# szpajder/dumpvdl2

Hardware: AMD Instinct MI355X
Metric: IQ MS/s demodulated end-to-end (higher is better)
Workload: dtype f32

## Files before the change

dumpvdl2_amd/csrc/kernels.h:

```cpp
#pragma once
#include <hip/hip_runtime.h>
#include <type_traits>
#include "vdl2_core.h"
#include "design.h"

#ifndef VDL2_K1_UNROLL
#define VDL2_K1_UNROLL 5
#endif

#ifndef VDL2_K1_WAVES_PER_EU
#define VDL2_K1_WAVES_PER_EU 3
#endif

namespace vdl2 {

constexpr int kK1Unroll = VDL2_K1_UNROLL;
typedef float v2f __attribute__((ext_vector_type(2)));
typedef float v4f __attribute__((ext_vector_type(4)));

#ifndef VDL2_REF_PRIO
#define VDL2_REF_PRIO 3
#endif
#ifndef VDL2_K1_PRIO
#define VDL2_K1_PRIO 0
// ... 789 lines not shown
			const float4 ts = seg ? a.seg_end[(size_t)c * a.nseg_cap + seg - 1] : a.carry_in[c];
			const float *Pp = bf.Ppow[len];
			e.x += Pp[0] * ts.x + Pp[1] * ts.z; e.y += Pp[0] * ts.y + Pp[1] * ts.w;
			e.z += Pp[2] * ts.x + Pp[3] * ts.z; e.w += Pp[2] * ts.y + Pp[3] * ts.w;
		}
		a.carry_out[c] = e;
	}
}

__global__ void k_carry(K1Args a, void *carry_out, uint32_t nrem) {
	const uint32_t i = threadIdx.x;
	if(i >= nrem) return;
	const int64_t s = (int64_t)(a.nlogical - nrem) + i;
	if(a.fmt == 1) {
		const uint32_t *p = (s < (int64_t)a.ncarry) ? (const uint32_t *)a.carry + s : (const uint32_t *)a.in + (s - a.ncarry);
		((uint32_t *)carry_out)[i] = *p;
	} else {
		const uint16_t *p = (s < (int64_t)a.ncarry) ? (const uint16_t *)a.carry + s : (const uint16_t *)a.in + (s - a.ncarry);
		((uint16_t *)carry_out)[i] = *p;
	}
}

__device__ __forceinline__ void reset_out_ctl(OutCtl *ctl, uint32_t k5_waves) {
	ctl->nbursts = 0; ctl->overflow = 0; ctl->nvalid = 0; ctl->pool_out_used = 0;
	ctl->nframes = burst_reserve_initial_frames(k5_waves); ctl->pool_used = burst_reserve_initial_pool(k5_waves);
}
__global__ void k_reset_ctl(OutCtl *ctl, uint32_t k5_waves) { reset_out_ctl(ctl, k5_waves); }

struct K3Args {
	const cf32 *y; cf32 *pf; uint64_t *cand; uint64_t *flag; const Tables *tab;
	int64_t nbase, k1;
	uint32_t cap, mask;
	int32_t wpl;
	OutCtl *ctl; uint32_t k5_waves;
	RefChan *ref; RefChan refv; float max_ppm; const float *ppm_thr; int32_t ref_on; uint32_t *rq_n, *rq_flag; RefBad *rq_bad; ScanReq *pq; uint32_t pq_cap; uint32_t *rq_flag2;
};

#ifndef VDL2_K3_SHARE
#define VDL2_K3_SHARE 8
#endif
constexpr int kK3Share = VDL2_K3_SHARE, kK3Threads = 320, kK3Tile = kK3Threads * kK3Share;
static_assert(kK3Tile == kK3Threads * kK3Share && kK3Tile % 64 == 0 && kK3Threads % 10 == 0 && (kK3Tile / 64) % (kK3Threads / 64) == 0, "screen tile");

__global__ __launch_bounds__(kK3Threads) void k_sync_screen(K3Args a) {
	if(blockIdx.x == 0 && blockIdx.y == 0 && threadIdx.x == 0 && a.rq_n) a.rq_n[3] = 0u;
	__shared__ float tile[kK3Tile + 150];
	__shared__ uint8_t verdict[kK3Tile];
	const int c = blockIdx.y, tid = threadIdx.x;
	const int64_t nblk = a.nbase + (int64_t)blockIdx.x * kK3Tile;
	const cf32 *y = a.y + (size_t)c * a.cap;
	constexpr int kFull = (kK3Tile + 150) / kK3Threads, kRest = (kK3Tile + 150) % kK3Threads;
	if(nblk >= 150 && nblk + kK3Tile <= a.k1) {
		const uint32_t r0 = (uint32_t)(nblk - 150) + tid;
		cf32 v[kFull + 1];
		#pragma unroll
		for(int k = 0; k <= kFull; k++) if(k < kFull || tid < kRest) v[k] = y[(r0 + kK3Threads * k) & a.mask];
		#pragma unroll
		for(int k = 0; k <= kFull; k++) if(k < kFull || tid < kRest) tile[tid + kK3Threads * k] = phase_fast(v[k]);
	} else {
		for(int j = tid; j < kK3Tile + 150; j += kK3Threads) {
			const int64_t t = nblk - 150 + j;
			tile[j] = (t < 0 || t >= a.k1) ? 0.f : phase_fast(y[(uint32_t)t & a.mask]);
		}
	}
	__syncthreads();
	const int s0 = 10 * kK3Share * (tid / 10) + tid % 10;
	constexpr int kEarlyPh = kScreenEarly + kK3Share - 1;
	float ph[kEarlyPh], d[kEarlyPh];
	#pragma unroll
	for(int k = 0; k < kEarlyPh; k++) ph[k] = tile[s0 + 10 * k];
	#pragma unroll
	for(int k = 1; k < kEarlyPh; k++) d[k] = ph[k] - ph[k - 1];
	#pragma unroll
	for(int q = 0; q < kK3Share; q++) {
		ScreenAcc acc;
		screen_begin(acc);
		screen_taps(&d[q], 1, kScreenEarly, acc);
		float ps = screen_value(acc, kScreenEarly);
		if(__any(ps < kScreenEarlyThr)) {
			float pl[kPreamble - kScreenEarly + 1], dl[kPreamble];
			#pragma unroll
			for(int j = 0; j <= kPreamble - kScreenEarly; j++) pl[j] = tile[s0 + 10 * (q + kScreenEarly - 1 + j)];
			#pragma unroll
			for(int j = 0; j < kPreamble - kScreenEarly; j++) dl[kScreenEarly + j] = pl[j + 1] - pl[j];
			screen_taps(dl, kScreenEarly, kPreamble, acc);
			ps = screen_value(acc, kPreamble);
		}
		verdict[s0 + 10 * q] = !(ps >= kScreenThr);
	}
	__syncthreads();
	#pragma unroll
	for(int j = 0; j < (kK3Tile / 64) / (kK3Threads / 64); j++) {
		const int word = (tid >> 6) * ((kK3Tile / 64) / (kK3Threads / 64)) + j;
		const int64_t n = nblk + 64 * word + (tid & 63);
		const unsigned long long bits = __ballot(n < a.k1 && verdict[64 * word + (tid & 63)] != 0);
		if((tid & 63) == 0 && n < a.k1) a.flag[(size_t)c * (a.cap >> 6) + ((uint32_t)(n >> 6) & (a.mask >> 6))] = bits;
	}
}

constexpr int kK3bWordsPerLane = 4;
template<bool FULL>
__global__ __launch_bounds__(256, 4) void k_sync_exact4(K3Args a) {
	if(blockIdx.x == 0 && blockIdx.y == 0 && threadIdx.x == 0) { reset_out_ctl(a.ctl, a.k5_waves); if(a.ref) *a.ref = a.refv; if(a.rq_n) { a.rq_n[0] = 0u; a.rq_n[1] = 0u; a.rq_n[2] = 0u; a.rq_n[4] = 0u; a.rq_n[5] = 0u; a.rq_n[6] = 0u; } }
	if(blockIdx.x == 0 && threadIdx.x == 0 && a.rq_flag) { a.rq_flag[blockIdx.y] = 0u; a.rq_bad[blockIdx.y].n = 0u; if(a.rq_flag2) a.rq_flag2[blockIdx.y] = 0u; }
	constexpr int kBack = 160, kSpan = kBack + 64;
	__shared__ float psh[4][64 + 6], fsh[4][64 + 6], esh[4][64 + 6], ash[4][64 + 6], bsh[4][64 + 6];
	__shared__ float phs[4][kSpan], e2s[4][kSpan];
	__shared__ uint64_t s_need[4][64 * kK3bWordsPerLane];
	__shared__ uint8_t s_fprev[4][64 * kK3bWordsPerLane];
	__shared__ uint16_t s_list[4][64 * kK3bWordsPerLane];
	const int c = blockIdx.y, lane = threadIdx.x & 63, wave = threadIdx.x >> 6;
	const cf32 *y = a.y + (size_t)c * a.cap;
	const uint64_t *flag = a.flag + (size_t)c * (a.cap >> 6);
	uint64_t *cand = a.cand + (size_t)c * (a.cap >> 6);
	const uint32_t wmask = a.mask >> 6;
	const Tables &T = *a.tab;
	const bool ref_on = a.ref != nullptr && a.ref_on != 0;
	const float ppm_thr = ref_on ? a.ppm_thr[c] : 0.f;
	const int64_t w0 = a.nbase >> 6, w1 = (a.k1 + 63) >> 6;
	const int64_t wb = w0 + ((int64_t)blockIdx.x * 4 + wave) * (64 * a.wpl);
	int nwork = 0;
	for(int g = 0; g < a.wpl; g++) {
		const int64_t w = wb + 64 * g + lane;
		uint64_t need = 0, fprev = 0, fpp = 0, f0 = 0;
		if(w < w1) {
			f0 = flag[(uint32_t)w & wmask];
			fprev = w > 0 ? flag[(uint32_t)(w - 1) & wmask] : 0ull;
			fpp = w > 1 ? flag[(uint32_t)(w - 2) & wmask] : 0ull;
			const uint64_t fnext = w + 1 < w1 ? flag[(uint32_t)(w + 1) & wmask] : 0ull;
			need = f0 | (f0 << 3) | (f0 >> 3) | (fprev >> 61) | (fnext << 61);
			const int64_t base = w << 6;
			if(a.k1 - 3 < base + 64) {
				const int64_t lo = a.k1 - 3 - base;
				need |= lo <= 0 ? ~0ull : (~0ull << lo);
			}
			if(a.k1 < base + 64) need &= (a.k1 - base <= 0) ? 0ull : (~0ull >> (64 - (a.k1 - base)));
			if(need == 0) cand[(uint32_t)w & wmask] = 0;
		}
		const uint64_t need_prev = fprev | (fprev << 3) | (fprev >> 3) | (fpp >> 61) | (f0 << 61);
		s_need[wave][64 * g + lane] = need; s_fprev[wave][64 * g + lane] = (uint8_t)(need_prev >> 58);
		const unsigned long long busy = __ballot(need != 0);
		if(need != 0) s_list[wave][nwork + __builtin_popcountll(busy & ((1ull << lane) - 1ull))] = (uint16_t)(64 * g + lane);
		nwork += __builtin_popcountll(busy);
	}
	WAVE_SYNC();
	float *ps = psh[wave], *fs = fsh[wave], *es = esh[wave], *as = ash[wave], *bs = bsh[wave], *ph = phs[wave], *e2 = e2s[wave];
	#pragma unroll 1
	for(int it = 0; it < nwork; it++) {
		const int idx = (int)s_list[wave][it];
		const uint64_t needj = s_need[wave][idx];
		const uint32_t fprevj = s_fprev[wave][idx] & 63u;
		const int64_t wj = wb + idx, r0 = (wj << 6) - kBack;
		{
			cf32 yv[4]; bool in[4];
			#pragma unroll
			for(int k = 0; k < 4; k++) {
				const int64_t t = r0 + lane + 64 * k;
				in[k] = 64 * k + lane < kSpan && t >= 0 && t < a.k1;
				yv[k] = in[k] ? y[(uint32_t)t & a.mask] : cf32{0.f, 0.f};
			}
			#pragma unroll
			for(int k = 0; k < 4; k++) if(64 * k + lane < kSpan) {
				ph[64 * k + lane] = in[k] ? phase_of(yv[k]) : 0.f;
				e2[64 * k + lane] = in[k] ? yv[k].re * yv[k].re + yv[k].im * yv[k].im : -1.f;
			}
		}
		ps[6 + lane] = kPherrBig; if(lane < 6) ps[lane] = kPherrBig;
		WAVE_SYNC();
		if(ref_on) {
			float ev[4];
			#pragma unroll
			for(int k = 0; k < 4; k++) {
				const int i = 64 * k + lane;
				ev[k] = 0.f;
				if(i >= 3 && i < kSpan) {
					const float m0 = e2[i], m1 = e2[i - 1], m2 = e2[i - 2], m3 = e2[i - 3];
					ev[k] = m0 < 0.f ? 0.f : ref_eps2_of(m0, fmaxf(m1, 0.f), fmaxf(m2, 0.f), fmaxf(m3, 0.f));
				}
			}
			WAVE_SYNC();
			#pragma unroll
			for(int k = 0; k < 4; k++) if(64 * k + lane < kSpan) e2[64 * k + lane] = ev[k];
			WAVE_SYNC();
		}
		#pragma unroll 1
		for(int round = 0; round < 2; round++) {
			const int bit = round == 0 ? lane : lane - 6;
			const bool todo = round == 0 ? ((needj >> lane) & 1ull) != 0 : (lane < 6 && ((fprevj >> lane) & 1u) && (wj << 6) + bit >= 0);
			if(todo) {
				const int i0 = bit + kBack - 150;
				float p[kPreamble];
				#pragma unroll
				for(int i = 0; i < kPreamble; i++) p[i] = ph[i0 + 10 * i];
				float pv, fv, E = 0.f, pa, pb;
				if(ref_on) sync_metric_ref(p, e2 + i0, 10, T, pv, fv, E, pa, pb, FULL);
				else { sync_metric(p, T, pv, fv); pa = pb = pv; }
				ps[6 + bit] = pv; fs[6 + bit] = fv; es[6 + bit] = E; as[6 + bit] = pa; bs[6 + bit] = pb;
			}
		}
		WAVE_SYNC();
		const int64_t n = (wj << 6) + lane;
		const float p0 = ps[6 + lane], p3 = ps[3 + lane], p6 = ps[lane];
		int vd = 0;
		if(n >= 3 && n < a.k1) {
			if(!ref_on) vd = is_candidate(p3, p0) ? 1 : 0;
			else vd = ref_candidate_verdict(ref_pherr_range(p0, as[6 + lane], bs[6 + lane], es[6 + lane]), ref_pherr_range(p3, as[3 + lane], bs[3 + lane], es[3 + lane]), fs[3 + lane], es[3 + lane],
			                                ref_pherr_range(p6, as[lane], bs[lane], es[lane]), a.max_ppm, ppm_thr);
		}
		if((needj >> lane) & 1ull) a.pf[(size_t)c * a.cap + ((uint32_t)n & a.mask)] = cf32{ (vd & 2) ? -p0 : p0, fs[6 + lane] };
		const unsigned long long bits = __ballot((vd & 1) != 0);
		if(lane == 0) cand[(uint32_t)wj & wmask] = bits;
		if(a.pq) {
			const unsigned long long mk = __ballot((vd & 2) != 0 && ((needj >> lane) & 1ull) != 0);
			if(mk && lane == 0) {
				const int64_t nf = (wj << 6) + __builtin_ctzll(mk), nl = (wj << 6) + 63 - __builtin_clzll(mk);
				int64_t lo = (nf - kRefPre) & ~255ll, hi = (nl + kRefPost) | 255; if(lo < 0) lo = 0; if(hi > a.k1 - 1) hi = a.k1 - 1;
				const uint32_t i = atomicAdd(a.rq_n + 3, 1u);
				if(i < a.pq_cap) a.pq[i] = ScanReq{ c, REF_CANDIDATE, lo, hi };
			}
		}
		WAVE_SYNC();
	}
}

struct K4Args {
	const cf32 *y; const cf32 *pf; const uint64_t *cand; const Tables *tab;
	WalkState *ws; unsigned long long *cnt; Burst *bursts; uint32_t *nb_chan; uint32_t cap_bursts_chan; OutCtl *ctl; const uint32_t *freq;
	EvalChunk *log; uint32_t *nlog; uint32_t cap_log;
	int64_t k_end; float max_ppm; uint32_t cap, mask; int32_t chan_first, nchan;
	const float *ppm_thr;
	RefChan *ref;
	uint32_t ref_launch;
	RefReq *rq; uint32_t *rq_n; uint32_t rq_cap; uint32_t *rq_flag; WalkState *ws_snap; unsigned long long *cnt_snap; RefBad *rq_bad; int32_t ref_pre;
	int32_t force_again;
	WalkState *ws_tmp; unsigned long long *cnt_tmp; WalkState *ws_snap_next; unsigned long long *cnt_snap_next; uint32_t *rq_flag2, *rq_flag2_next;
	int32_t force_mismatch;
};

__global__ __launch_bounds__(64, 4) void k_walk(K4Args a) {
	__shared__ WalkShared sh;
	const int c = blockIdx.x;
	ChanView v{ a.y + (size_t)c * a.cap, a.pf + (size_t)c * a.cap, a.cand + (size_t)c * (a.cap >> 6), a.mask, a.ref, c, a.ref_launch, a.rq, a.rq_n, a.rq_cap, a.rq_flag, a.rq_bad ? a.rq_bad + c : nullptr, a.ref_pre != 0 };
	EvalLog lg{ a.log + (size_t)c * a.cap_log, a.nlog + c };
	walk_channel(c, a.freq[c], a.max_ppm, a.ppm_thr[c], a.k_end, *a.tab, v, &a.ws[c], a.cnt + (size_t)c * kNumCounters,
	             a.bursts + (size_t)c * a.cap_bursts_chan, a.cap_bursts_chan, a.nb_chan + c, a.ctl, lg, sh, WalkSnap{ a.rq ? a.ws_snap : nullptr, a.cnt_snap });
}

__global__ __launch_bounds__(64, 4) void k_ref_verify(K4Args a) {
	__shared__ float lds[64];
	const uint32_t nreq = *a.rq_n < a.rq_cap ? *a.rq_n : a.rq_cap;
	if(a.force_again && blockIdx.x == 0) for(int c = (int)threadIdx.x; c < a.nchan; c += 64) a.rq_flag[c] = 1u;
	for(uint32_t i = blockIdx.x; i < nreq; i += gridDim.x) {
		const RefReq r = a.rq[i];
		const int c = r.chan;
		ChanView v{ a.y + (size_t)c * a.cap, a.pf + (size_t)c * a.cap, a.cand + (size_t)c * (a.cap >> 6), a.mask, a.ref, c, a.ref_launch + 2u };
// ... 576 lines not shown
```

dumpvdl2_amd/csrc/vdl2hip.hip:

```cpp
#include <hip/hip_runtime.h>
#include <hip/hip_ext.h>
#include <algorithm>
#include <cstdio>
#include <cstdlib>
#include <cstring>
#include <memory>
#include <mutex>
#include <new>
#include <string>
#include <vector>
#include "../../include/vdl2hip.h"
#include "kernels.h"
#include "tables.h"

using namespace vdl2;

static_assert(VDL2HIP_NUM_COUNTERS == kNumCounters, "counter enum out of sync");

namespace {

struct HostFrame {
	OutFrame f;
	std::shared_ptr<std::vector<uint8_t>> pool;
	const uint8_t *octets() const { return pool && f.pool_off + f.len <= pool->size() ? pool->data() + f.pool_off : nullptr; }
// ... 47 lines not shown
	vdl2hip_cfg cfg{};
	int C = 0, chan_first = 0, os = 0, fmt = 0, run = kRun, cr = 1;
	bool specialised = false;
	std::vector<uint32_t> freqs, dphi;
	LpfCoeffs lpf{};
	BlockForm bf{};
	hipStream_t stream = nullptr;
	BlockForm *d_bf = nullptr; Lut4 *d_lut = nullptr; Tables *d_tab = nullptr;
	uint32_t *d_dphi = nullptr, *d_freq = nullptr; float *d_ppmthr = nullptr;
	uint8_t *d_in[kSlots] = {}; hipEvent_t ev_copied[kSlots] = {}; size_t in_cap = 0;
	hipStream_t stream_copy = nullptr, stream_out = nullptr;
	hipEvent_t pinned_pending = nullptr;
	struct { int n = 0; uint64_t samples[kColdParts] = {}; hipEvent_t ev[kColdParts] = {}; } cold;
	uint8_t *h_stage = nullptr; size_t stage_cap = 0;
	uint8_t *d_carry[2] = {nullptr, nullptr}; int carry_sel = 0; uint32_t ncarry = 0;
	cf32 *d_y = nullptr, *d_pf = nullptr; uint64_t *d_cand = nullptr, *d_flag = nullptr;
	uint32_t cap = 0;
	float4 *d_segend = nullptr; uint32_t nseg_cap = 0;
	float4 *d_qpow = nullptr;
	float4 *d_tcarry[2] = {nullptr, nullptr}; int tcarry_sel = 0;
	unsigned long long *d_segpub = nullptr; uint32_t *d_synctmo = nullptr; bool fuse_k2 = true;
	WalkState *d_ws = nullptr; unsigned long long *d_cnt = nullptr, *d_acnt = nullptr;
	unsigned long long *d_wcnt = nullptr;
	NfState *d_nf = nullptr; int64_t *d_scfirst = nullptr, *d_sccum = nullptr;
	float *d_nfring = nullptr, *d_lpbuf = nullptr; NfFeed *d_nffeed = nullptr; uint32_t cap_log = 0, cap_comb = 0, cap_hist = 0, nf_ring = 0;
	uint32_t cap_bursts_chan = 0;
	SpecOut *d_spec[2] = {}; uint32_t *d_segstats = nullptr; int seg_max = 1; int64_t seg_min = 16384;
	OutSlot slot[kSlots];
	uint64_t feed_no = 0; int drain_lag = 0;
	hipStream_t stream_pre[kSidePre] = {};
	hipStream_t stream_back = nullptr, stream_nf = nullptr, stream_burst[kSideBurst] = {};
	OutCtl ctl_template{};
	bool pooled = false;
	bool avlc_filter = false, failed = false; int debug_force_timeout = 0, debug_force_again = 0;
	bool referee = true; bool ref_prescan = false;    int64_t ref_warm = 3 << 16 , ref_T = 0; uint8_t *d_refhist = nullptr; uint64_t ref_cap = 0, ref_wp = 0;
	struct HistPiece { int64_t s0, n; uint64_t pos; }; std::vector<HistPiece> ref_pieces;
	WalkState *d_ws_snap[2] = {}, *d_ws_tmp = nullptr; unsigned long long *d_cnt_snap[2] = {}, *d_cnt_tmp = nullptr; uint32_t rq_cap = 8192; uint32_t sq_alloc = 8192;
	int walk_ahead = 1; bool walk_ahead_auto = true; double walk_ahead_below = 1.1e8; int debug_force_mismatch = 0;
	int ref_retry_mul = 2;
	RefChan *d_ref[kSlots] = {}; unsigned long long *d_refdone = nullptr; uint32_t *d_refdonen = nullptr, *d_refstats = nullptr; uint8_t *d_mix = nullptr;
	std::vector<uint64_t> statsd_prev;
	std::vector<HostFrame> queue;
	int64_t k_total = 0; uint64_t n_total = 0;
	int profiling = 0;
	vdl2hip_stats stats{};
};

#define HIPCHK(expr) do { hipError_t e_ = (expr); if(e_ != hipSuccess) { \
	fprintf(stderr, "vdl2hip: %s failed: %s (%s:%d)\n", #expr, hipGetErrorString(e_), __FILE__, __LINE__); return VDL2HIP_E_DEVICE; } } while(0)

static size_t sample_bytes(int fmt) { return fmt == VDL2HIP_FMT_S16LE ? 4 : 2; }

struct OnDevice {
	int prev = -1; bool switched = false;
	explicit OnDevice(const vdl2hip_ctx *c) { if(c && hipGetDevice(&prev) == hipSuccess && prev != c->cfg.device) switched = hipSetDevice(c->cfg.device) == hipSuccess; }
	~OnDevice() { if(switched) (void)hipSetDevice(prev); }
};

#define LAUNCH_EV(kernel, grid, block, stream, e0, e1, ...) hipExtLaunchKernelGGL(kernel, grid, block, 0u, stream, e0, e1, 0, __VA_ARGS__)
#define EV(i) (prof_all ? ev[i] : (hipEvent_t) nullptr)

template<int OS, int R>
static void launch_chanfir(vdl2hip_ctx *c, const K1Args &a, int cr, size_t lds, hipEvent_t e0, hipEvent_t e1) {
	const int groups = (c->C + cr - 1) / cr;
	K1Args b = a;
	b.gy = (groups + 3) / 4;
	const int nseg8 = (a.seg1 - a.seg0 + 7) / 8 * 8;
// ... 163 lines not shown
		refv.done = c->d_refdone; refv.done_n = c->d_refdonen; refv.stats = c->d_refstats;
		int np = 0;
		const int64_t blk_s0 = (int64_t)c->n_total, want0 = blk_s0 - c->ref_T;
		for(size_t i = c->ref_pieces.size() > 2 ? c->ref_pieces.size() - 2 : 0; i < c->ref_pieces.size(); i++) {
			vdl2hip_ctx::HistPiece hp = c->ref_pieces[i];
			if(hp.s0 + hp.n <= want0) continue;
			if(hp.s0 < want0) { hp.pos = (hp.pos + (uint64_t)(want0 - hp.s0)) % c->ref_cap; hp.n -= want0 - hp.s0; hp.s0 = want0; }
			const uint64_t first = std::min<uint64_t>((uint64_t)hp.n, c->ref_cap - hp.pos);
			refv.piece[np++] = RefPiece{ c->d_refhist + hp.pos * sb, hp.s0, (int64_t)first };
			if(first < (uint64_t)hp.n) refv.piece[np++] = RefPiece{ c->d_refhist, hp.s0 + (int64_t)first, hp.n - (int64_t)first };
		}
		refv.piece[np++] = RefPiece{ dev_in, blk_s0, (int64_t)nnew };
		refv.npiece = np;
		int firstp = 0;
		for(int i = 1; i < np; i++) if(refv.piece[i - 1].s0 + refv.piece[i - 1].n != refv.piece[i].s0) firstp = i;
		if(firstp) { for(int i = firstp; i < np; i++) refv.piece[i - firstp] = refv.piece[i]; refv.npiece = np - firstp; }
		if(nnew) {
			const uint64_t w = std::min<uint64_t>(nnew, (uint64_t)c->ref_T);
			hipLaunchKernelGGL(k_ref_hist, dim3((unsigned)((w + 255) / 256)), dim3(256), 0, st, (const uint8_t *)dev_in + (nnew - w) * sb, w, c->d_refhist, c->ref_wp, c->ref_cap, (int)sb);
			if(w < nnew) c->ref_pieces.clear();
			if(!c->ref_pieces.empty() && c->ref_pieces.back().s0 + c->ref_pieces.back().n == blk_s0 + (int64_t)(nnew - w)) c->ref_pieces.back().n += (int64_t)w;
			else c->ref_pieces.push_back(vdl2hip_ctx::HistPiece{ blk_s0 + (int64_t)(nnew - w), (int64_t)w, c->ref_wp });
			c->ref_wp = (c->ref_wp + w) % c->ref_cap;
			auto &bp = c->ref_pieces.back();
			if((uint64_t)bp.n > c->ref_cap / 2) { const int64_t cut = bp.n - (int64_t)(c->ref_cap / 2); bp.s0 += cut; bp.pos = (bp.pos + (uint64_t)cut) % c->ref_cap; bp.n -= cut; }
			while(c->ref_pieces.size() > 2) c->ref_pieces.erase(c->ref_pieces.begin());
		}
	}
	if(D > 0) {
		const int64_t k1 = c->k_total + D, nbase = c->k_total & ~63ll;
		sl.k5_waves = (unsigned)std::min<int64_t>(2048, std::max<int64_t>(16, (D * (int64_t)c->C) >> 14));
		sl.k5_waves = (sl.k5_waves + kBurstWaves - 1) / kBurstWaves * kBurstWaves;
		sl.prescan = c->referee && c->ref_prescan && !feed_is_small(c, D);
		K3Args k3{ c->d_y, c->d_pf, c->d_cand, c->d_flag, c->d_tab, nbase, k1, c->cap, c->cap - 1, 1, sl.d_ctl, sl.k5_waves, ref_dst, refv, c->cfg.max_ppm, c->d_ppmthr, c->referee ? 1 : 0, sl.d_rqn, sl.d_rqflag, sl.d_rqbad, sl.prescan ? sl.d_pq : nullptr, kPreScans, sl.d_rqflag2 };
		LAUNCH_EV(k_sync_screen, dim3((unsigned)((k1 - nbase + kK3Tile - 1) / kK3Tile), (unsigned)c->C), dim3(kK3Threads), st, EV(4), (hipEvent_t) nullptr, k3);
		const int64_t nwords = ((k1 + 63) >> 6) - (nbase >> 6);
		for(int wpl = kK3bWordsPerLane; wpl >= 1; wpl >>= 1) { k3.wpl = wpl; if(((nwords + 256 * wpl - 1) / (256 * wpl)) * c->C >= 2048 || wpl == 1) break; }
		const int64_t wpb = 256 * k3.wpl;
		if(c->referee && c->ref_prescan) LAUNCH_EV(k_sync_exact4<true>, dim3((unsigned)((nwords + wpb - 1) / wpb), (unsigned)c->C), dim3(256), st, (hipEvent_t) nullptr, sl.ev_front, k3);
		else LAUNCH_EV(k_sync_exact4<false>, dim3((unsigned)((nwords + wpb - 1) / wpb), (unsigned)c->C), dim3(256), st, (hipEvent_t) nullptr, sl.ev_front, k3);
	}
	if(D <= 0) HIPCHK(hipEventRecord(sl.ev_front, st));
	if(D > 0) { sl.ev_valid = prof; sl.ev_level = c->profiling; sl.fused = a.fuse != 0; if(sl.k1_timed) c->stats.chan_samples += (uint64_t)D * c->os * c->C; } else sl.k1_timed = false;
	sl.back_D = D; sl.back_k0 = c->k_total;
	sl.pending = true; sl.seq = c->feed_no++;
	c->k_total += D; c->n_total += nnew;
	c->stats.feeds++; c->stats.input_samples += nnew;
	{ int r = launch_back(c, sl); if(r != VDL2HIP_OK) return r; }
	HIPCHK(hipGetLastError());
	return VDL2HIP_OK;
}

static bool feed_is_small(const vdl2hip_ctx *c, int64_t D) {
	const int nseg = (int)std::min<int64_t>(c->seg_max, D / c->seg_min);
	return D > 0 && D < 2 * c->seg_min && nseg < 2;
}
#define LAUNCH_SCAN_MULTI(how, ...) do { \
	if(c->fmt == 1) { if(c->os == 20) how((k_ref_scan_multi<1, 20>), __VA_ARGS__); else if(c->os == 10) how((k_ref_scan_multi<1, 10>), __VA_ARGS__); else how((k_ref_scan_multi<1, 0>), __VA_ARGS__); } \
	else { if(c->os == 20) how((k_ref_scan_multi<0, 20>), __VA_ARGS__); else if(c->os == 10) how((k_ref_scan_multi<0, 10>), __VA_ARGS__); else how((k_ref_scan_multi<0, 0>), __VA_ARGS__); } } while(0)
static void launch_scans(vdl2hip_ctx *c, hipStream_t st, RefChan *ref, uint32_t launch, const ScanReq *sq, const RefReq *rq, const uint32_t *n, uint32_t cap, int64_t k_end,
                         ScanReq *retry, uint32_t *retry_n, hipEvent_t e0 = nullptr, hipEvent_t e1 = nullptr) {
	const int rty = retry ? c->ref_retry_mul : 0;
	LAUNCH_SCAN_MULTI(hipExtLaunchKernelGGL, dim3((cap + kScanLanes - 1) / kScanLanes), dim3(64 * kScanWaves), 0, st, e0, rty ? (hipEvent_t) nullptr : e1, 0, ref, launch,
	                  sq, rq, n, cap, k_end, rty ? retry : (ScanReq *) nullptr, retry_n, kRetryScans, 1);
	if(rty) LAUNCH_SCAN_MULTI(hipExtLaunchKernelGGL, dim3(kRetryScans / kScanLanes), dim3(64 * kScanWaves), 0, st, (hipEvent_t) nullptr, e1, 0, ref, launch,
	                  (const ScanReq *)retry, (const RefReq *) nullptr, (const uint32_t *)retry_n, kRetryScans, k_end, (ScanReq *) nullptr, (uint32_t *) nullptr, 0u, rty);
}
static int launch_rest(vdl2hip_ctx *c, OutSlot &sl, OutSlot *succ);
static void launch_stitch(vdl2hip_ctx *c, hipStream_t st, const OutSlot &sl, const K4Args &k4, int again, hipEvent_t e1 = nullptr) {
	K4sArgs k4s{ k4, sl.d_spec_of, (uint32_t)(3 * (c->seg_max - 1)), sl.nseg, sl.back_k0, sl.seglen, c->d_segstats, again };
	hipExtLaunchKernelGGL(k_walk_stitch, dim3((unsigned)((c->C + kStitchWaves - 1) / kStitchWaves)), dim3(64 * kStitchWaves), (unsigned)(sizeof(StitchLds) * kStitchWaves), st, (hipEvent_t) nullptr, e1, 0, k4s);
}

// ... 654 lines not shown
		if(hipMemcpy(&tmo, c->d_synctmo, 4, hipMemcpyDeviceToHost) != hipSuccess) return VDL2HIP_E_DEVICE;
		c->stats.front_sync_timeouts = tmo;
		for(int i = 0; i < c->C; i++) { c->stats.seg_adopted += ss[2 * i]; c->stats.seg_walked += ss[2 * i + 1]; }
	}
	if(c->d_refstats) {
		uint32_t rs[11] = {0, 0, 0, 0, 0, 0, 0, 0, 0, 0, 0};
		if(hipMemcpy(rs, c->d_refstats, sizeof rs, hipMemcpyDeviceToHost) != hipSuccess) return VDL2HIP_E_DEVICE;
		c->stats.referee_scans = rs[0]; c->stats.referee_cached = rs[1]; c->stats.referee_refused = rs[2]; c->stats.referee_short = rs[3];
		c->stats.referee_candidate_scans = rs[4]; c->stats.referee_header_scans = rs[5]; c->stats.referee_symbol_scans = rs[6]; c->stats.referee_rewalks = rs[7]; c->stats.referee_redone_next = rs[8]; c->stats.referee_unmet = rs[9]; c->stats.referee_retried = rs[10];
	}
	memcpy(out, &c->stats, std::min(size, sizeof c->stats));
	return (r == VDL2HIP_E_OVERFLOW || c->failed) ? VDL2HIP_OK : r;
}
int vdl2hip_get_stats(vdl2hip_ctx *c, vdl2hip_stats *out) { return vdl2hip_get_stats_sized(c, out, sizeof(vdl2hip_stats)); }

void *vdl2hip_stream(vdl2hip_ctx *c) { return c ? (void *)c->stream : nullptr; }

int vdl2hip_set_drain_lag(vdl2hip_ctx *c, int lag) {
	if(!c || lag < 0 || lag > kSlots - 1) return VDL2HIP_E_INVAL;
	c->drain_lag = lag;
	return VDL2HIP_OK;
}

int vdl2hip_debug_option(vdl2hip_ctx *c, const char *name, long value) {
	if(!c || !name) return VDL2HIP_E_INVAL;
	OnDevice dev_guard(c);
	int r = collect_pending(c);
	if(r != VDL2HIP_OK && r != VDL2HIP_E_OVERFLOW) return r;
	if(strcmp(name, "no_fuse") == 0) { c->fuse_k2 = value == 0; return VDL2HIP_OK; }
	if(strcmp(name, "force_timeout") == 0) { c->debug_force_timeout = value != 0; return VDL2HIP_OK; }
	if(strcmp(name, "force_mismatch") == 0) { c->debug_force_mismatch = value != 0; return VDL2HIP_OK; }
	if(strcmp(name, "walk_ahead_below") == 0) { c->walk_ahead_below = (double)value; c->walk_ahead_auto = true; return VDL2HIP_OK; }
	if(strcmp(name, "walk_ahead") == 0) { if(value != 0 && value != 1) return VDL2HIP_E_INVAL; c->walk_ahead = (int)value; c->walk_ahead_auto = false; return VDL2HIP_OK; }
	if(strcmp(name, "force_again") == 0) { c->debug_force_again = value != 0; return VDL2HIP_OK; }
	if(strcmp(name, "referee") == 0) { if(value && !c->d_refhist) return VDL2HIP_E_INVAL; c->referee = value != 0; return VDL2HIP_OK; }
	if(strcmp(name, "ref_warm") == 0) { if(value < 0 || value > c->ref_T - 4096) return VDL2HIP_E_INVAL; c->ref_warm = value; return VDL2HIP_OK; }
	return VDL2HIP_E_INVAL;
}

int vdl2hip_debug_exact_window_many(vdl2hip_ctx *c, uint32_t chan, int64_t n_lo, int64_t n_hi, uint32_t count, int64_t stride, float *ms) {
	if(!c || !c->d_refhist || chan >= (uint32_t)c->C || c->feed_no == 0 || count == 0 || count > 65536) return VDL2HIP_E_INVAL;
	OnDevice dev_guard(c);
	int r = collect_pending(c);
	if(r != VDL2HIP_OK && r != VDL2HIP_E_OVERFLOW) return r;
	int *d_out = nullptr; std::vector<int> h(count, 0);
	if(hipMalloc((void **)&d_out, 4 * (size_t)count) != hipSuccess) return VDL2HIP_E_NOMEM;
	hipEvent_t e0 = nullptr, e1 = nullptr;
	bool ok = hipEventCreate(&e0) == hipSuccess && hipEventCreate(&e1) == hipSuccess;
	if(ok) hipExtLaunchKernelGGL(k_ref_probe, dim3(count), dim3(64), 0, c->stream, e0, e1, 0, c->d_ref[(c->feed_no - 1) % kSlots], (int)chan, c->C, n_lo, n_hi, stride, d_out);
	ok = ok && hipStreamSynchronize(c->stream) == hipSuccess && hipMemcpy(h.data(), d_out, 4 * (size_t)count, hipMemcpyDeviceToHost) == hipSuccess;
	float t = 0.f;
	if(ok && ms) { (void)hipEventElapsedTime(&t, e0, e1); *ms = t; }
	if(e0) (void)hipEventDestroy(e0);
	if(e1) (void)hipEventDestroy(e1);
	(void)hipFree(d_out);
	if(!ok) return VDL2HIP_E_DEVICE;
	int n = 0; for(int v : h) n += v;
	return n;
}
int vdl2hip_debug_scan_multi2(vdl2hip_ctx *c, const int32_t *chan, const int64_t *lo, const int64_t *hi, uint32_t count, int with_retry, float *ms) {
	if(!c || !c->d_refhist || c->feed_no == 0 || count == 0 || count > 65536 || !chan || !lo || !hi) return VDL2HIP_E_INVAL;
	OnDevice dev_guard(c);
	int r = collect_pending(c);
	if(r != VDL2HIP_OK && r != VDL2HIP_E_OVERFLOW) return r;
	std::vector<ScanReq> h(count);
	for(uint32_t i = 0; i < count; i++) { if(chan[i] < 0 || chan[i] >= c->C) return VDL2HIP_E_INVAL; h[i] = ScanReq{ chan[i], REF_CANDIDATE, lo[i], hi[i] }; }
// ... 23 lines not shown

int vdl2hip_debug_u8_levels(float out[512]) {
	float *d = nullptr;
	if(hipMalloc((void **)&d, 512 * sizeof(float)) != hipSuccess) return VDL2HIP_E_NOMEM;
	hipLaunchKernelGGL(k_u8_level_probe, dim3(1), dim3(256), 0, 0, d);
	const bool ok = hipMemcpy(out, d, 512 * sizeof(float), hipMemcpyDeviceToHost) == hipSuccess;
	(void)hipFree(d);
	return ok ? VDL2HIP_OK : VDL2HIP_E_DEVICE;
}

int vdl2hip_debug_dpp_probe(const float in[64], float out[256]) {
	float *d_in = nullptr, *d_out = nullptr;
	if(hipMalloc((void **)&d_in, 64 * 4) != hipSuccess || hipMalloc((void **)&d_out, 256 * 4) != hipSuccess) return VDL2HIP_E_NOMEM;
	int rc = VDL2HIP_OK;
	if(hipMemcpy(d_in, in, 64 * 4, hipMemcpyHostToDevice) != hipSuccess) rc = VDL2HIP_E_DEVICE;
	if(rc == VDL2HIP_OK) {
		hipLaunchKernelGGL(k_dpp_probe, dim3(1), dim3(64), 0, 0, (const float *)d_in, d_out);
		if(hipMemcpy(out, d_out, 256 * 4, hipMemcpyDeviceToHost) != hipSuccess) rc = VDL2HIP_E_DEVICE;
	}
	(void)hipFree(d_in); (void)hipFree(d_out);
	return rc;
}

#ifdef VDL2_K1_PROF
int vdl2hip_debug_k1_prof(unsigned long long out[16], int reset) {
	static unsigned long long h[64][16];
	if(hipMemcpyFromSymbol(h, HIP_SYMBOL(vdl2_k1_prof), sizeof h) != hipSuccess) return -3;
	for(int k = 0; k < 16; k++) { out[k] = 0; for(int s = 0; s < 64; s++) out[k] += h[s][k]; }
	if(reset) { memset(h, 0, sizeof h); if(hipMemcpyToSymbol(HIP_SYMBOL(vdl2_k1_prof), h, sizeof h) != hipSuccess) return -3; }
	return 0;
}
#endif

#ifdef VDL2_K5_PROF
int vdl2hip_debug_k5_prof(unsigned long long out[16], int reset) {
	static unsigned long long h[64][16];
	if(hipMemcpyFromSymbol(h, HIP_SYMBOL(vdl2_k5_prof), sizeof h) != hipSuccess) return -3;
	for(int k = 0; k < 16; k++) { out[k] = 0; for(int s = 0; s < 64; s++) out[k] += h[s][k]; }
	if(reset) { memset(h, 0, sizeof h); if(hipMemcpyToSymbol(HIP_SYMBOL(vdl2_k5_prof), h, sizeof h) != hipSuccess) return -3; }
	return 0;
}
int vdl2hip_debug_nf_prof(unsigned long long out[16], int reset) {
	static unsigned long long h[64][16];
	if(hipMemcpyFromSymbol(h, HIP_SYMBOL(vdl2_nf_prof), sizeof h) != hipSuccess) return -3;
	for(int k = 0; k < 16; k++) { out[k] = 0; for(int s = 0; s < 64; s++) out[k] += h[s][k]; }
	if(reset) { memset(h, 0, sizeof h); if(hipMemcpyToSymbol(HIP_SYMBOL(vdl2_nf_prof), h, sizeof h) != hipSuccess) return -3; }
	return 0;
}
int vdl2hip_debug_k4_prof(unsigned long long out[24], int reset) {
	static unsigned long long h[64][24];
	if(hipMemcpyFromSymbol(h, HIP_SYMBOL(vdl2_k4_prof), sizeof h) != hipSuccess) return -3;
	for(int k = 0; k < 24; k++) { out[k] = 0; for(int s = 0; s < 64; s++) out[k] += h[s][k]; }
	if(reset) { memset(h, 0, sizeof h); if(hipMemcpyToSymbol(HIP_SYMBOL(vdl2_k4_prof), h, sizeof h) != hipSuccess) return -3; }
	return 0;
}
#endif

int vdl2hip_get_lpf(vdl2hip_ctx *c, float A[3], float B[3]) {
	if(!c) return VDL2HIP_E_INVAL;
	memcpy(A, c->lpf.A, sizeof c->lpf.A); memcpy(B, c->lpf.B, sizeof c->lpf.B);
	return VDL2HIP_OK;
}

int vdl2hip_get_nco_step(vdl2hip_ctx *c, uint32_t chan, uint32_t *dphi) {
	if(!c || !dphi || chan < (uint32_t)c->chan_first || chan >= (uint32_t)(c->chan_first + c->C)) return VDL2HIP_E_INVAL;
	*dphi = nco_step(c->cfg.centerfreq, c->freqs[chan - c->chan_first], (uint32_t)kSymbolRate * kSps * c->os);
// ... 49 lines not shown
```

Baseline: 4753.

## Add dense block-wide sync evaluation kernel replacing per-wave word-serial exact pass

```diff
diff --git a/dumpvdl2_amd/csrc/kernels.h b/dumpvdl2_amd/csrc/kernels.h
--- a/dumpvdl2_amd/csrc/kernels.h
+++ b/dumpvdl2_amd/csrc/kernels.h
@@ -845,6 +845,7 @@
 	int64_t nbase, k1;
 	uint32_t cap, mask;
 	int32_t wpl;
+	int32_t screen_all;
 	OutCtl *ctl; uint32_t k5_waves;
 	RefChan *ref; RefChan refv; float max_ppm; const float *ppm_thr; int32_t ref_on; uint32_t *rq_n, *rq_flag; RefBad *rq_bad; ScanReq *pq; uint32_t pq_cap; uint32_t *rq_flag2;
 };
@@ -906,12 +907,26 @@
 	for(int j = 0; j < (kK3Tile / 64) / (kK3Threads / 64); j++) {
 		const int word = (tid >> 6) * ((kK3Tile / 64) / (kK3Threads / 64)) + j;
 		const int64_t n = nblk + 64 * word + (tid & 63);
-		const unsigned long long bits = __ballot(n < a.k1 && verdict[64 * word + (tid & 63)] != 0);
+		const unsigned long long bits = __ballot(n < a.k1 && (verdict[64 * word + (tid & 63)] != 0 || a.screen_all != 0));
 		if((tid & 63) == 0 && n < a.k1) a.flag[(size_t)c * (a.cap >> 6) + ((uint32_t)(n >> 6) & (a.mask >> 6))] = bits;
 	}
 }
 
 constexpr int kK3bWordsPerLane = 4;
+#ifdef VDL2_K3B_PROF
+__device__ unsigned long long vdl2_k3b_prof[64][16];
+#define K3B_BEGIN() unsigned k3b_t0_ = (unsigned)__builtin_readcyclecounter(), k3b_acc_[6] = {0, 0, 0, 0, 0, 0}, k3b_cnt_[3] = {0, 0, 0}
+#define K3B_MARK(k) do { if(__builtin_amdgcn_readfirstlane(threadIdx.x >> 6) == 0) { const unsigned t_ = (unsigned)__builtin_readcyclecounter(); \
+	k3b_acc_[k] += t_ - k3b_t0_; k3b_t0_ = t_; } } while(0)
+#define K3B_COUNT(k, v) do { k3b_cnt_[k] += (unsigned)__builtin_amdgcn_readfirstlane((int)(v)); } while(0)
+#define K3B_END() do { if(threadIdx.x == 0) { const int s_ = (blockIdx.x + blockIdx.y) & 63; for(int k_ = 0; k_ < 6; k_++) atomicAdd(&vdl2_k3b_prof[s_][k_], (unsigned long long)k3b_acc_[k_]); \
+	atomicAdd(&vdl2_k3b_prof[s_][8], 1ull); for(int k_ = 0; k_ < 3; k_++) atomicAdd(&vdl2_k3b_prof[s_][9 + k_], (unsigned long long)k3b_cnt_[k_]); } } while(0)
+#else
+#define K3B_BEGIN() do {} while(0)
+#define K3B_MARK(k) do {} while(0)
+#define K3B_COUNT(k, v) do {} while(0)
+#define K3B_END() do {} while(0)
+#endif
 template<bool FULL>
 __global__ __launch_bounds__(256, 4) void k_sync_exact4(K3Args a) {
 	if(blockIdx.x == 0 && blockIdx.y == 0 && threadIdx.x == 0) { reset_out_ctl(a.ctl, a.k5_waves); if(a.ref) *a.ref = a.refv; if(a.rq_n) { a.rq_n[0] = 0u; a.rq_n[1] = 0u; a.rq_n[2] = 0u; a.rq_n[4] = 0u; a.rq_n[5] = 0u; a.rq_n[6] = 0u; } }
@@ -933,6 +948,7 @@
 	const int64_t w0 = a.nbase >> 6, w1 = (a.k1 + 63) >> 6;
 	const int64_t wb = w0 + ((int64_t)blockIdx.x * 4 + wave) * (64 * a.wpl);
 	int nwork = 0;
+	K3B_BEGIN();
 	for(int g = 0; g < a.wpl; g++) {
 		const int64_t w = wb + 64 * g + lane;
 		uint64_t need = 0, fprev = 0, fpp = 0, f0 = 0;
@@ -957,6 +973,7 @@
 		nwork += __builtin_popcountll(busy);
 	}
 	WAVE_SYNC();
+	K3B_MARK(0); if(wave == 0) K3B_COUNT(0, nwork);
 	float *ps = psh[wave], *fs = fsh[wave], *es = esh[wave], *as = ash[wave], *bs = bsh[wave], *ph = phs[wave], *e2 = e2s[wave];
 	#pragma unroll 1
 	for(int it = 0; it < nwork; it++) {
@@ -980,6 +997,7 @@
 		}
 		ps[6 + lane] = kPherrBig; if(lane < 6) ps[lane] = kPherrBig;
 		WAVE_SYNC();
+		K3B_MARK(1); if(wave == 0) { K3B_COUNT(1, __builtin_popcountll(needj) + __builtin_popcount(fprevj)); K3B_COUNT(2, 1 + (fprevj != 0)); }
 		if(ref_on) {
 			float ev[4];
 			#pragma unroll
@@ -996,6 +1014,7 @@
 			for(int k = 0; k < 4; k++) if(64 * k + lane < kSpan) e2[64 * k + lane] = ev[k];
 			WAVE_SYNC();
 		}
+		K3B_MARK(2);
 		#pragma unroll 1
 		for(int round = 0; round < 2; round++) {
 			const int bit = round == 0 ? lane : lane - 6;
@@ -1010,6 +1029,7 @@
 				else { sync_metric(p, T, pv, fv); pa = pb = pv; }
 				ps[6 + bit] = pv; fs[6 + bit] = fv; es[6 + bit] = E; as[6 + bit] = pa; bs[6 + bit] = pb;
 			}
+			K3B_MARK(3 + round);
 		}
 		WAVE_SYNC();
 		const int64_t n = (wj << 6) + lane;
@@ -1033,7 +1053,210 @@
 			}
 		}
 		WAVE_SYNC();
-	}
+		K3B_MARK(5);
+	}
+	K3B_END();
+}
+
+constexpr int kK3dEvals = 320;
+constexpr int kK3dFlush = kK3dEvals - 64;
+constexpr int kK3dList = kK3dFlush + 256;
+constexpr int kK3dMinGroups = 2048;
+constexpr int kK3dGroup = 4;
+constexpr int kK3dRounds = 32;
+static_assert(kK3dEvals >= 70 && kK3dEvals <= 512 && kK3dList * 70 < (1 << 20) && kK3dList < (1 << 11) && kK3dRounds * 256 <= (1 << 16),
+              "tile map: 9 bits of word, 7 of position; list head: 11 bits of words, 21 of evaluations; 16 bits of word index");
+#define K3D_BARRIER() do { __builtin_amdgcn_fence(__ATOMIC_RELEASE, "workgroup", "local"); __builtin_amdgcn_s_barrier(); __builtin_amdgcn_fence(__ATOMIC_ACQUIRE, "workgroup", "local"); } while(0)
+template<bool FULL>
+__global__ __launch_bounds__(256, 4) void k_sync_dense(K3Args a) {
+	if(blockIdx.x == 0 && blockIdx.y == 0 && threadIdx.x == 0) { reset_out_ctl(a.ctl, a.k5_waves); if(a.ref) *a.ref = a.refv; if(a.rq_n) { a.rq_n[0] = 0u; a.rq_n[1] = 0u; a.rq_n[2] = 0u; a.rq_n[4] = 0u; a.rq_n[5] = 0u; a.rq_n[6] = 0u; } }
+	if(blockIdx.x == 0 && threadIdx.x == 0 && a.rq_flag) { a.rq_flag[blockIdx.y] = 0u; a.rq_bad[blockIdx.y].n = 0u; if(a.rq_flag2) a.rq_flag2[blockIdx.y] = 0u; }
+	__shared__ uint64_t s_need[kK3dList], s_cbits[kK3dList], s_mbits[kK3dList];
+	__shared__ uint32_t s_end[kK3dList];
+	__shared__ uint16_t s_word[kK3dList];
+	__shared__ uint8_t s_fprev[kK3dList];
+	__shared__ uint16_t s_map[kK3dEvals];
+	__shared__ float s_res[5][kK3dEvals];
+	__shared__ uint8_t s_neg[kK3dEvals];
+	__shared__ uint32_t s_head, s_r1;
+	__shared__ uint64_t s_flag[256 * kK3dGroup + 3];
+	const int c = blockIdx.y, tid = threadIdx.x, lane = threadIdx.x & 63;
+	const cf32 *y = a.y + (size_t)c * a.cap;
+	const uint64_t *flag = a.flag + (size_t)c * (a.cap >> 6);
+	uint64_t *cand = a.cand + (size_t)c * (a.cap >> 6);
+	const uint32_t wmask = a.mask >> 6;
+	const Tables &T = *a.tab;
+	const bool ref_on = a.ref != nullptr && a.ref_on != 0;
+	const float ppm_thr = ref_on ? a.ppm_thr[c] : 0.f;
+	const int64_t w0 = a.nbase >> 6, w1 = (a.k1 + 63) >> 6;
+	const int64_t wb = w0 + (int64_t)blockIdx.x * (256 * a.wpl);
+	K3B_BEGIN();
+	if(tid == 0) s_head = 0u;
+	K3D_BARRIER();
+	#pragma unroll 1
+	for(int g = 0; g < a.wpl; g++) {
+		if(g % kK3dGroup == 0) {
+			const int ng = a.wpl - g < kK3dGroup ? a.wpl - g : kK3dGroup;
+			for(int i = tid; i < 256 * ng + 3; i += 256) {
+				const int64_t w = wb + 256 * g - 2 + i;
+				s_flag[i] = w >= 0 && w < w1 ? flag[(uint32_t)w & wmask] : 0ull;
+			}
+			K3D_BARRIER();
+		}
+		{
+			const int64_t w = wb + 256 * g + tid;
+			const int fi = 256 * (g % kK3dGroup) + tid;
+			uint64_t need = 0, fprev = 0, fpp = 0, f0 = 0;
+			if(w < w1) {
+				f0 = s_flag[fi + 2]; fprev = s_flag[fi + 1]; fpp = s_flag[fi];
+				const uint64_t fnext = s_flag[fi + 3];
+				need = f0 | (f0 << 3) | (f0 >> 3) | (fprev >> 61) | (fnext << 61);
+				const int64_t base = w << 6;
+				if(a.k1 - 3 < base + 64) {
+					const int64_t lo = a.k1 - 3 - base;
+					need |= lo <= 0 ? ~0ull : (~0ull << lo);
+				}
+				if(a.k1 < base + 64) need &= (a.k1 - base <= 0) ? 0ull : (~0ull >> (64 - (a.k1 - base)));
+				if(need == 0) cand[(uint32_t)w & wmask] = 0;
+			}
+			const uint64_t need_prev = fprev | (fprev << 3) | (fprev >> 3) | (fpp >> 61) | (f0 << 61);
+			const uint32_t fp6 = w > 0 ? (uint32_t)(need_prev >> 58) : 0u;
+			const uint32_t cnt = need != 0 ? (uint32_t)__builtin_popcountll(need) + (uint32_t)__builtin_popcount(fp6) : 0u;
+			const uint32_t inc = cnt << 11 | (need != 0 ? 1u : 0u);
+			uint32_t incl = inc;
+			#pragma unroll
+			for(int d = 1; d < 64; d <<= 1) { const uint32_t o = (uint32_t)__shfl_up((int)incl, d); if(lane >= d) incl += o; }
+			const uint32_t tot = (uint32_t)__shfl((int)incl, 63);
+			uint32_t at = 0;
+			if(lane == 0 && tot != 0) at = atomicAdd(&s_head, tot);
+			at = (uint32_t)__shfl((int)at, 0) + incl - inc;
+			if(need != 0) {
+				const uint32_t r = at & 2047u;
+				s_need[r] = need; s_fprev[r] = (uint8_t)fp6; s_word[r] = (uint16_t)(256 * g + tid); s_end[r] = (at >> 11) + cnt;
+				s_cbits[r] = 0ull; s_mbits[r] = 0ull;
+			}
+		}
+		K3D_BARRIER();
+		const uint32_t head = s_head;
+		K3D_BARRIER();
+		const int nrec = (int)(head & 2047u);
+		K3B_MARK(0);
+		if((int)(head >> 11) < kK3dFlush && g + 1 < a.wpl) continue;
+		K3B_COUNT(0, nrec); K3B_COUNT(1, head >> 11);
+		#pragma unroll 1
+		for(int r0 = 0; r0 < nrec; ) {
+			const uint32_t e0 = r0 ? s_end[r0 - 1] : 0u;
+			if(tid == 0) s_r1 = (uint32_t)r0 + 1u;
+			K3D_BARRIER();
+			{
+				uint32_t best = 0;
+				for(int r = r0 + 1 + tid; r < nrec && r < r0 + kK3dEvals; r += 256) if(s_end[r] - e0 <= (uint32_t)kK3dEvals) best = (uint32_t)r + 1u;
+				if(best) atomicMax(&s_r1, best);
+			}
+			K3D_BARRIER();
+			const int r1 = (int)s_r1, nev = (int)(s_end[r1 - 1] - e0);
+			for(int r = r0 + tid; r < r1; r += 256) {
+				uint32_t at = (r ? s_end[r - 1] : 0u) - e0;
+				const uint32_t code = (uint32_t)(r - r0) << 7;
+				for(uint32_t m = s_fprev[r]; m; m &= m - 1u) s_map[at++] = (uint16_t)(code | (uint32_t)__builtin_ctz(m));
+				for(uint64_t m = s_need[r]; m; m &= m - 1ull) s_map[at++] = (uint16_t)(code | (6u + (uint32_t)__builtin_ctzll(m)));
+			}
+			K3D_BARRIER();
+			K3B_MARK(1); K3B_COUNT(2, 1);
+			#pragma unroll 1
+			for(int s = tid; s < nev; s += 256) {
+				const uint32_t code = s_map[s];
+				const int64_t n = ((wb + s_word[r0 + (int)(code >> 7)]) << 6) + (int)(code & 127u) - 6;
+				float p[kPreamble], e2[kPreamble];
+				cf32 yt[kPreamble];
+				#pragma unroll
+				for(int i = 0; i < kPreamble; i++) { const int64_t t = n - 150 + 10 * i; yt[i] = t >= 0 ? y[(uint32_t)t & a.mask] : cf32{0.f, 0.f}; }
+				if(ref_on) {
+					#pragma unroll
+					for(int h = 0; h < kPreamble; h += 4) {
+						cf32 yv[4][3];
+						#pragma unroll
+						for(int i = 0; i < 4; i++) {
+							#pragma unroll
+							for(int k = 0; k < 3; k++) { const int64_t t = n - 150 + 10 * (h + i) - 1 - k; yv[i][k] = t >= 0 ? y[(uint32_t)t & a.mask] : cf32{0.f, 0.f}; }
+						}
+						#pragma unroll
+						for(int i = 0; i < 4; i++) {
+							const int64_t t = n - 150 + 10 * (h + i);
+							float m[4];
+							m[0] = t >= 0 ? yt[h + i].re * yt[h + i].re + yt[h + i].im * yt[h + i].im : -1.f;
+							#pragma unroll
+							for(int k = 0; k < 3; k++) m[1 + k] = t - 1 - k >= 0 ? yv[i][k].re * yv[i][k].re + yv[i][k].im * yv[i][k].im : -1.f;
+							e2[h + i] = m[0] < 0.f ? 0.f : ref_eps2_of(m[0], fmaxf(m[1], 0.f), fmaxf(m[2], 0.f), fmaxf(m[3], 0.f));
+						}
+					}
+				}
+				#pragma unroll
+				for(int i = 0; i < kPreamble; i++) { const int64_t t = n - 150 + 10 * i; p[i] = t >= 0 ? phase_of(yt[i]) : 0.f; }
+				float pv, fv, E = 0.f, pa, pb;
+				if(ref_on) sync_metric_ref(p, e2, 1, T, pv, fv, E, pa, pb, FULL);
+				else { sync_metric(p, T, pv, fv); pa = pb = pv; }
+				s_res[0][s] = pv; s_res[1][s] = fv; s_res[2][s] = E; s_res[3][s] = pa; s_res[4][s] = pb; s_neg[s] = 0;
+			}
+			K3D_BARRIER();
+			K3B_MARK(3);
+			#pragma unroll 1
+			for(int s = tid; s < nev; s += 256) {
+				const uint32_t code = s_map[s];
+				const int r = r0 + (int)(code >> 7), pos = (int)(code & 127u) + 3;
+				if(pos < 6 || pos > 69) continue;
+				const uint64_t needj = s_need[r];
+				const uint64_t mlo = (uint64_t)s_fprev[r] | (needj << 6), mhi = needj >> 58;
+				const int at = (int)((r ? s_end[r - 1] : 0u) - e0);
+				const int64_t n = ((wb + s_word[r]) << 6) + pos - 6;
+				if(!(n >= 3 && n < a.k1)) continue;
+				int sl[2];
+				#pragma unroll
+				for(int k = 0; k < 2; k++) {
+					const int q = pos - 6 * k;
+					const bool has = q < 64 ? ((mlo >> q) & 1ull) != 0 : ((mhi >> (q - 64)) & 1ull) != 0;
+					const int below = q < 64 ? __builtin_popcountll(mlo & ((1ull << q) - 1ull)) : __builtin_popcountll(mlo) + __builtin_popcountll(mhi & ((1ull << (q - 64)) - 1ull));
+					sl[k] = has ? at + below : -1;
+				}
+				const int i0 = sl[0] < 0 ? 0 : sl[0], i6 = sl[1] < 0 ? 0 : sl[1];
+				const bool h0 = sl[0] >= 0, h6 = sl[1] >= 0;
+				const float p0 = h0 ? s_res[0][i0] : kPherrBig, p3 = s_res[0][s], p6 = h6 ? s_res[0][i6] : kPherrBig;
+				int vd;
+				if(!ref_on) vd = is_candidate(p3, p0) ? 1 : 0;
+				else vd = ref_candidate_verdict(ref_pherr_range(p0, h0 ? s_res[3][i0] : 0.f, h0 ? s_res[4][i0] : 0.f, h0 ? s_res[2][i0] : 0.f), ref_pherr_range(p3, s_res[3][s], s_res[4][s], s_res[2][s]), s_res[1][s], s_res[2][s],
+				                                ref_pherr_range(p6, h6 ? s_res[3][i6] : 0.f, h6 ? s_res[4][i6] : 0.f, h6 ? s_res[2][i6] : 0.f), a.max_ppm, ppm_thr);
+				if(vd & 1) atomicOr((unsigned long long *)&s_cbits[r], 1ull << (pos - 6));
+				if((vd & 2) && h0) { atomicOr((unsigned long long *)&s_mbits[r], 1ull << (pos - 6)); s_neg[i0] = 1; }
+			}
+			K3D_BARRIER();
+			#pragma unroll 1
+			for(int s = tid; s < nev; s += 256) {
+				const uint32_t code = s_map[s];
+				const int pos = (int)(code & 127u);
+				if(pos < 6) continue;
+				const int64_t n = ((wb + s_word[r0 + (int)(code >> 7)]) << 6) + pos - 6;
+				const float p0 = s_res[0][s];
+				a.pf[(size_t)c * a.cap + ((uint32_t)n & a.mask)] = cf32{ s_neg[s] ? -p0 : p0, s_res[1][s] };
+			}
+			for(int r = r0 + tid; r < r1; r += 256) {
+				const int64_t wj = wb + s_word[r];
+				cand[(uint32_t)wj & wmask] = s_cbits[r];
+				const uint64_t mk = s_mbits[r];
+				if(a.pq && mk) {
+					const int64_t nf = (wj << 6) + __builtin_ctzll(mk), nl = (wj << 6) + 63 - __builtin_clzll(mk);
+					int64_t lo = (nf - kRefPre) & ~255ll, hi = (nl + kRefPost) | 255; if(lo < 0) lo = 0; if(hi > a.k1 - 1) hi = a.k1 - 1;
+					const uint32_t i = atomicAdd(a.rq_n + 3, 1u);
+					if(i < a.pq_cap) a.pq[i] = ScanReq{ c, REF_CANDIDATE, lo, hi };
+				}
+			}
+			K3D_BARRIER();
+			K3B_MARK(5);
+			r0 = r1;
+		}
+		if(tid == 0) s_head = 0u;
+		K3D_BARRIER();
+	}
+	K3B_END();
 }
 
 struct K4Args {
diff --git a/dumpvdl2_amd/csrc/vdl2hip.hip b/dumpvdl2_amd/csrc/vdl2hip.hip
--- a/dumpvdl2_amd/csrc/vdl2hip.hip
+++ b/dumpvdl2_amd/csrc/vdl2hip.hip
@@ -103,7 +103,7 @@
 	hipStream_t stream_back = nullptr, stream_nf = nullptr, stream_burst[kSideBurst] = {};
 	OutCtl ctl_template{};
 	bool pooled = false;
-	bool avlc_filter = false, failed = false; int debug_force_timeout = 0, debug_force_again = 0;
+	bool avlc_filter = false, failed = false; int debug_force_timeout = 0, debug_force_again = 0, debug_exact_tier = 1, debug_screen_all = 0;
 	bool referee = true; bool ref_prescan = false;    int64_t ref_warm = 3 << 16 , ref_T = 0; uint8_t *d_refhist = nullptr; uint64_t ref_cap = 0, ref_wp = 0;
 	struct HistPiece { int64_t s0, n; uint64_t pos; }; std::vector<HistPiece> ref_pieces;
 	WalkState *d_ws_snap[2] = {}, *d_ws_tmp = nullptr; unsigned long long *d_cnt_snap[2] = {}, *d_cnt_tmp = nullptr; uint32_t rq_cap = 8192; uint32_t sq_alloc = 8192;
@@ -333,13 +333,22 @@
 		sl.k5_waves = (unsigned)std::min<int64_t>(2048, std::max<int64_t>(16, (D * (int64_t)c->C) >> 14));
 		sl.k5_waves = (sl.k5_waves + kBurstWaves - 1) / kBurstWaves * kBurstWaves;
 		sl.prescan = c->referee && c->ref_prescan && !feed_is_small(c, D);
-		K3Args k3{ c->d_y, c->d_pf, c->d_cand, c->d_flag, c->d_tab, nbase, k1, c->cap, c->cap - 1, 1, sl.d_ctl, sl.k5_waves, ref_dst, refv, c->cfg.max_ppm, c->d_ppmthr, c->referee ? 1 : 0, sl.d_rqn, sl.d_rqflag, sl.d_rqbad, sl.prescan ? sl.d_pq : nullptr, kPreScans, sl.d_rqflag2 };
+		K3Args k3{ c->d_y, c->d_pf, c->d_cand, c->d_flag, c->d_tab, nbase, k1, c->cap, c->cap - 1, 1, c->debug_screen_all, sl.d_ctl, sl.k5_waves, ref_dst, refv, c->cfg.max_ppm, c->d_ppmthr, c->referee ? 1 : 0, sl.d_rqn, sl.d_rqflag, sl.d_rqbad, sl.prescan ? sl.d_pq : nullptr, kPreScans, sl.d_rqflag2 };
 		LAUNCH_EV(k_sync_screen, dim3((unsigned)((k1 - nbase + kK3Tile - 1) / kK3Tile), (unsigned)c->C), dim3(kK3Threads), st, EV(4), (hipEvent_t) nullptr, k3);
 		const int64_t nwords = ((k1 + 63) >> 6) - (nbase >> 6);
 		for(int wpl = kK3bWordsPerLane; wpl >= 1; wpl >>= 1) { k3.wpl = wpl; if(((nwords + 256 * wpl - 1) / (256 * wpl)) * c->C >= 2048 || wpl == 1) break; }
+		if(c->debug_exact_tier) {
+			for(int wpl = kK3dRounds; wpl >= 1; wpl >>= 1) { k3.wpl = wpl; if(((nwords + 256 * wpl - 1) / (256 * wpl)) * c->C >= kK3dMinGroups || wpl == 1) break; }
+		}
 		const int64_t wpb = 256 * k3.wpl;
-		if(c->referee && c->ref_prescan) LAUNCH_EV(k_sync_exact4<true>, dim3((unsigned)((nwords + wpb - 1) / wpb), (unsigned)c->C), dim3(256), st, (hipEvent_t) nullptr, sl.ev_front, k3);
-		else LAUNCH_EV(k_sync_exact4<false>, dim3((unsigned)((nwords + wpb - 1) / wpb), (unsigned)c->C), dim3(256), st, (hipEvent_t) nullptr, sl.ev_front, k3);
+		const dim3 k3b_grid((unsigned)((nwords + wpb - 1) / wpb), (unsigned)c->C);
+		if(c->debug_exact_tier) {
+			if(c->referee && c->ref_prescan) LAUNCH_EV(k_sync_dense<true>, k3b_grid, dim3(256), st, (hipEvent_t) nullptr, sl.ev_front, k3);
+			else LAUNCH_EV(k_sync_dense<false>, k3b_grid, dim3(256), st, (hipEvent_t) nullptr, sl.ev_front, k3);
+		} else {
+			if(c->referee && c->ref_prescan) LAUNCH_EV(k_sync_exact4<true>, k3b_grid, dim3(256), st, (hipEvent_t) nullptr, sl.ev_front, k3);
+			else LAUNCH_EV(k_sync_exact4<false>, k3b_grid, dim3(256), st, (hipEvent_t) nullptr, sl.ev_front, k3);
+		}
 	}
 	if(D <= 0) HIPCHK(hipEventRecord(sl.ev_front, st));
 	if(D > 0) { sl.ev_valid = prof; sl.ev_level = c->profiling; sl.fused = a.fuse != 0; if(sl.k1_timed) c->stats.chan_samples += (uint64_t)D * c->os * c->C; } else sl.k1_timed = false;
@@ -1060,6 +1069,8 @@
 	if(strcmp(name, "force_mismatch") == 0) { c->debug_force_mismatch = value != 0; return VDL2HIP_OK; }
 	if(strcmp(name, "walk_ahead_below") == 0) { c->walk_ahead_below = (double)value; c->walk_ahead_auto = true; return VDL2HIP_OK; }
 	if(strcmp(name, "walk_ahead") == 0) { if(value != 0 && value != 1) return VDL2HIP_E_INVAL; c->walk_ahead = (int)value; c->walk_ahead_auto = false; return VDL2HIP_OK; }
+	if(strcmp(name, "exact_tier") == 0) { if(value != 0 && value != 1) return VDL2HIP_E_INVAL; c->debug_exact_tier = (int)value; return VDL2HIP_OK; }
+	if(strcmp(name, "screen_all") == 0) { c->debug_screen_all = value != 0; return VDL2HIP_OK; }
 	if(strcmp(name, "force_again") == 0) { c->debug_force_again = value != 0; return VDL2HIP_OK; }
 	if(strcmp(name, "referee") == 0) { if(value && !c->d_refhist) return VDL2HIP_E_INVAL; c->referee = value != 0; return VDL2HIP_OK; }
 	if(strcmp(name, "ref_warm") == 0) { if(value < 0 || value > c->ref_T - 4096) return VDL2HIP_E_INVAL; c->ref_warm = value; return VDL2HIP_OK; }
@@ -1149,6 +1160,16 @@
 }
 #endif
 
+#ifdef VDL2_K3B_PROF
+int vdl2hip_debug_k3b_prof(unsigned long long out[16], int reset) {
+	static unsigned long long h[64][16];
+	if(hipMemcpyFromSymbol(h, HIP_SYMBOL(vdl2_k3b_prof), sizeof h) != hipSuccess) return -3;
+	for(int k = 0; k < 16; k++) { out[k] = 0; for(int s = 0; s < 64; s++) out[k] += h[s][k]; }
+	if(reset) { memset(h, 0, sizeof h); if(hipMemcpyToSymbol(HIP_SYMBOL(vdl2_k3b_prof), h, sizeof h) != hipSuccess) return -3; }
+	return 0;
+}
+#endif
+
 #ifdef VDL2_K5_PROF
 int vdl2hip_debug_k5_prof(unsigned long long out[16], int reset) {
 	static unsigned long long h[64][16];
```

Result: faster. 5068 (median of 6 runs) (+6.6%).
